# samuelkriegerbonini-dev/AstroBurst

Hardware: AMD Instinct MI355X
Metric: MPix/s sigma-clipped stack+stretch, 64x4096x4096 f32 (higher is better)
Workload: dtype f32

## Files before the change

astroburst_amd/csrc/tile_stream.hpp:

```cpp
#pragma once
#include <hip/hip_runtime.h>

#include <cstdint>

#include "ab_common.hpp"
#include "tile_bucket.hpp"

namespace ts {

using tb::dev_key;
using tb::wave_scan_incl;
using tb::wave_sort64;
using tb::Window;

constexpr int kThreads = 256;
constexpr int kWaves = kThreads / 64;
constexpr int kBuckets = 4096;
constexpr int kTop = kBuckets - 1;
constexpr int kPer = kBuckets / kThreads;
constexpr int kHotCap = 3072;
constexpr int kTabCap = 384;
constexpr int kSelCap = 1024;
constexpr int kMaxZones = 16;
constexpr int kRing = 2;
constexpr int kRingPlan = 3;
constexpr int kEdgePlan = 12;
#ifndef TS_PER_SIGMA
#define TS_PER_SIGMA 480.0f
#endif
constexpr float kPerSigma = TS_PER_SIGMA;
constexpr unsigned int kNone = 0xffffffffu;

enum Decline {
    D_NONE = 0, D_ZONES, D_HOT_OVERFLOW, D_MED_CATCHALL, D_MED_COLD, D_MED_BIG, D_DEV_BM, D_DEV_NOFIRST, D_DEV_SHAPE, D_DEV_COLD,
    D_DEV_BIG, D_DEV_COUNT, D_DEV_PROOF, D_EDGE_COLD, D_EDGE_CATCHALL, D_SAMPLE
};

struct alignas(16) Shared {
    unsigned int prefix[kBuckets + kThreads];
    float list[kHotCap + kThreads];
    union {
        unsigned char lut[kBuckets];
        unsigned int tmp[kSelCap];
    };
    unsigned int zcur[kMaxZones + kThreads];
    uint32_t tab_first[kTabCap], tab_last[kTabCap];
    unsigned int part[4 * kWaves];
    unsigned int zone_at[kMaxZones + 1];
    int zone_lo[kMaxZones], zone_hi[kMaxZones];
    int zone_tab[kMaxZones];
    int nzones;
    int decline;
    unsigned int ncand;
#ifdef AB_TILE_TIMING
    long long t_phase[16];
    long long t_mark;
#endif
};

#ifdef AB_TILE_TIMING
#define TS_MARK(sh, i)                             \
    do {                                           \
        if (threadIdx.x == 0) {                    \
            const long long now_ = clock64();      \
            (sh).t_phase[i] += now_ - (sh).t_mark; \
            (sh).t_mark = now_;                    \
        }                                          \
    } while (0)
#else
#define TS_MARK(sh, i) \
    do {               \
    } while (0)
#endif

__device__ __forceinline__ uint32_t ord_of(float x) {
    const uint32_t b = __float_as_uint(x);
    return b ^ ((b >> 31) ? 0xffffffffu : 0x80000000u);
}
__device__ __forceinline__ float from_ord(uint32_t u) { return __uint_as_float(u ^ ((u >> 31) ? 0x80000000u : 0xffffffffu)); }

struct Geo {
    float scale, off;
    float r_min, r_max;
    ab_pixel_xf xf;
    double range;
    __device__ __forceinline__ int bucket(float v) const { return (int)__builtin_amdgcn_fmed3f(__builtin_fmaf(v, scale, off), 0.0f, (float)kTop); }
    __device__ __forceinline__ bool is_cand(float v) const { return v >= r_min && v <= r_max; }
    __device__ __forceinline__ uint32_t norm_key(float raw) const { return __float_as_uint(ab_px(xf, raw)); }
    __device__ __forceinline__ float unnorm(float x) const { return xf.on ? (float)((double)x * range + xf.lo) : x; }
    __device__ __forceinline__ int bucket_at_norm(float x) const { return bucket(unnorm(x)); }
    __device__ __forceinline__ bool first_raw(int b, float *out) const {
        uint32_t u = ord_of(((float)b - off) / scale);
        int guard = 0;
        while (bucket(from_ord(u)) >= b && ++guard < 64) --u;
        while (bucket(from_ord(u)) < b && ++guard < 128) ++u;
        *out = from_ord(u);
        return guard < 128 && bucket(from_ord(u)) >= b && bucket(from_ord(u - 1u)) < b;
    }
    __device__ __forceinline__ bool first_norm(int b, uint32_t *key) const {
        if (b <= 0) {
            *key = 0x33d6bf96u;
            return true;
        }
        float r;
        if (!first_raw(b, &r)) return false;
        *key = norm_key(r < r_min ? r_min : r);
        return true;
    }
    __device__ __forceinline__ bool last_norm(int b, uint32_t *key) const {
        if (b >= kTop) {
            *key = norm_key(r_max);
            return true;
        }
        float r;
        if (!first_raw(b + 1, &r)) return false;
        r = from_ord(ord_of(r) - 1u);
        *key = norm_key(r < r_min ? r_min : r);
        return true;
    }
};

__device__ __forceinline__ void scan_prefix(Shared &sh) {
    const int t = threadIdx.x, b0 = t * kPer, w = t >> 6, lane = t & 63;
    unsigned int v[kPer];
#pragma unroll
    for (int j = 0; j < kPer; j += 4) {
        const uint4 q = *reinterpret_cast<const uint4 *>(&sh.prefix[b0 + j]);
        v[j] = q.x;
        v[j + 1] = q.y;
        v[j + 2] = q.z;
        v[j + 3] = q.w;
    }
#pragma unroll
    for (int j = 1; j < kPer; ++j) v[j] += v[j - 1];
    const unsigned int tot = v[kPer - 1], incl = wave_scan_incl(tot);
    if (lane == 63) sh.part[w] = incl;
    __syncthreads();
    unsigned int before = incl - tot;
#pragma unroll
    for (int i = 0; i < kWaves; ++i) before += i < w ? sh.part[i] : 0u;
#pragma unroll
    for (int j = 0; j < kPer; j += 4) {
        uint4 q;
        q.x = v[j] + before;
        q.y = v[j + 1] + before;
        q.z = v[j + 2] + before;
        q.w = v[j + 3] + before;
        *reinterpret_cast<uint4 *>(&sh.prefix[b0 + j]) = q;
    }
    __syncthreads();
}

__device__ __forceinline__ void wave_sync() { __builtin_amdgcn_fence(__ATOMIC_ACQ_REL, "wavefront"); }
__device__ __forceinline__ int first_lane(unsigned long long m) { return (int)__builtin_ctzll(m); }
__device__ __forceinline__ unsigned int lanes_below(unsigned long long m) {
    return __builtin_amdgcn_mbcnt_hi((unsigned int)(m >> 32), __builtin_amdgcn_mbcnt_lo((unsigned int)m, 0u));
}
__device__ __forceinline__ unsigned int below(const Shared &sh, int b) { return b <= 0 ? 0u : sh.prefix[b - 1]; }

__device__ __forceinline__ int wfind_rank(const Shared &sh, unsigned int g) {
    const int lane = threadIdx.x & 63;
    const unsigned long long m1 = __builtin_amdgcn_ballot_w64(g < sh.prefix[64 * lane + 63]);
    const int L = m1 ? first_lane(m1) : 63;
    const unsigned long long m2 = __builtin_amdgcn_ballot_w64(g < sh.prefix[64 * L + lane]);
    return 64 * L + (m2 ? first_lane(m2) : 63);
}

__device__ __forceinline__ unsigned int wprefix(const Shared &sh, const Window &w, int b) {
    const unsigned int p = below(sh, b);
    const unsigned int q = p < w.c_lo ? w.c_lo : (p > w.c_le_hi ? w.c_le_hi : p);
    return q - w.c_lo;
}

struct ZReg {
    int lo, hi, tab;
    unsigned int at, end;
    int n;
    __device__ __forceinline__ void load(const Shared &sh) {
        const int lane = threadIdx.x & 63;
        n = sh.nzones;
        const bool have = lane < n;
        lo = have ? sh.zone_lo[lane] : 0;
        hi = have ? sh.zone_hi[lane] : -1;
        tab = have ? sh.zone_tab[lane] : -1;
        at = have ? sh.zone_at[lane] : 0u;
        end = have ? sh.zone_at[lane + 1] : 0u;
    }
    __device__ __forceinline__ int zone_of(int b) const {
        const unsigned long long m = __builtin_amdgcn_ballot_w64(b >= lo && b <= hi);
        return m ? first_lane(m) : -1;
    }
    __device__ __forceinline__ int lo_of(int z) const { return __builtin_amdgcn_readlane(lo, z); }
    __device__ __forceinline__ int hi_of(int z) const { return __builtin_amdgcn_readlane(hi, z); }
    __device__ __forceinline__ unsigned int at_of(int z) const { return (unsigned int)__builtin_amdgcn_readlane((int)at, z); }
    __device__ __forceinline__ unsigned int end_of(int z) const { return (unsigned int)__builtin_amdgcn_readlane((int)end, z); }
    __device__ __forceinline__ int tab_index(int b) const {
        const unsigned long long m = __builtin_amdgcn_ballot_w64(tab >= 0 && b >= lo - 1 && b <= hi + 1);
        if (!m) return -1;
        const int z = first_lane(m);
        return __builtin_amdgcn_readlane(tab, z) + (b - __builtin_amdgcn_readlane(lo, z) + 1);
    }
};
__device__ __forceinline__ bool tfirst(const Shared &sh, const ZReg &zr, const Geo &g, int b, uint32_t *key) {
    const int i = zr.tab_index(b);
    if (i < 0) return g.first_norm(b, key);
    *key = sh.tab_first[i];
    return *key != 0u;
}
__device__ __forceinline__ bool tlast(const Shared &sh, const ZReg &zr, const Geo &g, int b, uint32_t *key) {
    const int i = zr.tab_index(b);
    if (i < 0) return g.last_norm(b, key);
    *key = sh.tab_last[i];
    return *key != 0u;
}

struct DevGeo {
    float mf;
    float delta;
    int bm;
};
__device__ __forceinline__ void ring_of(const Geo &g, const DevGeo &d, float t, int *bl, int *br) {
    const int l = g.bucket_at_norm(d.mf - t), r = g.bucket_at_norm(d.mf + t);
    *bl = l < d.bm ? l : d.bm;
    *br = r > d.bm ? r : d.bm;
}
__device__ __forceinline__ bool make_devgeo(const Shared &sh, const ZReg &zr, const Geo &g, double median, DevGeo *d) {
    d->mf = (float)median;
    int b = g.bucket_at_norm(d->mf), guard = 0;
    uint32_t k;
    auto first_le = [&](int bb, bool *le) {
        if (!tfirst(sh, zr, g, bb, &k)) return false;
        *le = (double)__uint_as_float(k) <= median;
        return true;
    };
    bool le;
    while (b > 0) {
        if (!first_le(b, &le)) return false;
        if (le || ++guard > 8) break;
        --b;
    }
    while (b < kTop) {
        if (!first_le(b + 1, &le)) return false;
        if (!le || ++guard > 16) break;
        ++b;
    }
    d->bm = b;
    if (b <= 0 || b >= kTop || guard > 16) return false;
    uint32_t k0, k1;
    if (!tfirst(sh, zr, g, b, &k0) || !tfirst(sh, zr, g, b + 1, &k1)) return false;
    d->delta = __uint_as_float(k1) - __uint_as_float(k0);
    return d->delta > 0.0f;
}

__device__ __forceinline__ unsigned int wmad_first(const Shared &sh, const Geo &g, const Window &w, const DevGeo &d, unsigned int need, unsigned int guess) {
    const int lane = threadIdx.x & 63;
    auto reaches = [&](unsigned int i) {
        int bl, br;
        ring_of(g, d, (float)(i + 1u) * d.delta, &bl, &br);
        return wprefix(sh, w, br + 1) - wprefix(sh, w, bl) >= need;
    };
    if (guess != kNone) {
        const unsigned int gi = guess < 3900u ? guess : 3900u, i_lo = gi > 96u ? gi - 96u : 0u;
#pragma unroll 1
        for (int j = 0; j < 4; ++j) {
            const unsigned long long m = __builtin_amdgcn_ballot_w64(reaches(i_lo + 64u * j + lane));
            if (m) {
                const unsigned int first = i_lo + 64u * j + (unsigned int)first_lane(m);
                if (first > i_lo || i_lo == 0u) return first;
                break;
            }
        }
    }
#pragma unroll 1
    for (int j = 0; j < kBuckets / 64; ++j) {
        const unsigned long long m = __builtin_amdgcn_ballot_w64(reaches(64u * j + lane));
        if (m) return 64u * j + (unsigned int)first_lane(m);
    }
    return kNone;
}

__device__ __forceinline__ int plan_zones(Shared &sh, const Geo &g, unsigned int cnt, float mad_guess, unsigned int (&first_guess)[3]) {
    int nz = 0;
    auto add = [&](int lo, int hi) {
        lo = lo < 1 ? 1 : lo;
        hi = hi > kTop - 1 ? kTop - 1 : hi;
        if (lo <= hi && nz < kMaxZones) {
            if ((threadIdx.x & 63) == 0) {
                sh.zone_lo[nz] = lo;
                sh.zone_hi[nz] = hi;
            }
            ++nz;
        }
    };
    Window w;
    w.lo = 1;
    w.hi = 0x7f7fffffu;
    w.c_lo = 0;
    w.c_le_hi = cnt;
    w.n = cnt;
    first_guess[0] = first_guess[1] = first_guess[2] = kNone;
#pragma unroll 1
    for (int it = 0; it < 3; ++it) {
        if (w.n < 3) break;
        const unsigned int mid = w.n / 2, g_hi = w.c_lo + mid, g_lo = w.n % 2 == 0 ? g_hi - 1 : g_hi;
        const int b_hi = wfind_rank(sh, g_hi), b_lo = g_lo == g_hi ? b_hi : wfind_rank(sh, g_lo);
        add(b_lo - 1, b_hi + 1);
        if (b_hi <= 0 || b_hi >= kTop) break;
        uint32_t k0, k1;
        if (!g.first_norm(b_hi, &k0) || !g.first_norm(b_hi + 1, &k1)) break;
        const unsigned int ex = below(sh, b_hi), in_b = sh.prefix[b_hi] - ex;
        const float frac = ((float)(g_hi - ex) + 0.5f) / (float)(in_b ? in_b : 1u);
        const float v0 = __uint_as_float(k0), v1 = __uint_as_float(k1);
        const double med = (double)(v0 + frac * (v1 - v0));
        DevGeo d;
        d.mf = (float)med;
        d.bm = b_hi;
        d.delta = v1 - v0;
        if (!(d.delta > 0.0f)) break;
        unsigned int guess = kNone;
        if (it == 0) {
            if (mad_guess > 0.0f) {
                const float gi = mad_guess / d.delta;
                guess = gi < 3900.0f ? (unsigned int)gi : 3900u;
            }
        } else {
            guess = first_guess[it - 1];
        }
        const unsigned int first = wmad_first(sh, g, w, d, mid + 1u, guess);
        if (first == kNone) break;
        first_guess[it] = first;
        {
            int bLo, bRo, bLi = d.bm, bRi = d.bm;
            ring_of(g, d, (float)(first + 1u + kRing + kRingPlan) * d.delta, &bLo, &bRo);
            if (first + 1u > (unsigned int)(kRing + kRingPlan)) ring_of(g, d, (float)(first + 1u - kRing - kRingPlan) * d.delta, &bLi, &bRi);
            if (bLi + 1 >= bRi) {
                add(bLo, bRo);
            } else {
                add(bLo, bLi);
                add(bRi, bRo);
            }
        }
        if (it == 2) break;
        const double mad = (double)(((float)first + 0.5f) * d.delta);
        const double sig = fmax(mad * 1.4826, 1e-30);
        const float lo = (float)(med - 3.0 * sig), hi = (float)(med + 3.0 * sig);
        if (!(lo <= hi)) break;
        const float e = (float)kEdgePlan * d.delta;
        int bl = 0, bh = kTop;
        if (lo > 0.0f) {
            add(g.bucket_at_norm(lo - e), g.bucket_at_norm(lo + e));
            bl = g.bucket_at_norm(lo);
        }
        if (hi < 3.0e38f) {
            add(g.bucket_at_norm(hi - e), g.bucket_at_norm(hi + e));
            bh = g.bucket_at_norm(hi);
        }
        unsigned int c_lo = lo > 0.0f ? below(sh, bl) + (sh.prefix[bl] - below(sh, bl)) / 2u : 0u;
        unsigned int c_hi = hi < 3.0e38f ? sh.prefix[bh] - (sh.prefix[bh] - below(sh, bh)) / 2u : cnt;
        c_lo = c_lo > w.c_lo ? c_lo : w.c_lo;
        c_hi = c_hi < w.c_le_hi ? c_hi : w.c_le_hi;
        if (c_hi <= c_lo) break;
        w.c_lo = c_lo;
        w.c_le_hi = c_hi;
        w.n = c_hi - c_lo;
    }
    return nz;
}

__device__ __forceinline__ bool build_zones(Shared &sh, const Geo &g, int nz) {
    const int lane = threadIdx.x & 63;
    wave_sync();
    uint32_t key = lane < nz ? ((uint32_t)sh.zone_lo[lane] << 16) | (uint32_t)sh.zone_hi[lane] : kNone;
    key = wave_sort64(key);
    int m = 0, cur_lo = 0, cur_hi = -2;
    int my_lo = 0, my_hi = -1;
    for (int i = 0; i < nz; ++i) {
        const uint32_t k = (uint32_t)__builtin_amdgcn_readlane((int)key, i);
        const int lo = (int)(k >> 16), hi = (int)(k & 0xffffu);
        if (m > 0 && lo <= cur_hi + 1) {
            cur_hi = hi > cur_hi ? hi : cur_hi;
        } else {
            if (m > 0 && lane == m - 1) {
                my_lo = cur_lo;
                my_hi = cur_hi;
            }
            cur_lo = lo;
            cur_hi = hi;
            ++m;
        }
    }
    if (m > 0 && lane == m - 1) {
        my_lo = cur_lo;
        my_hi = cur_hi;
    }
    const unsigned int size = lane < m ? sh.prefix[my_hi] - below(sh, my_lo) : 0u;
    const unsigned int tlen = lane < m ? (unsigned int)(my_hi - my_lo + 3) : 0u;
    const unsigned int at = wave_scan_incl(size) - size, tat = wave_scan_incl(tlen) - tlen;
    if (lane < m) {
        sh.zone_lo[lane] = my_lo;
        sh.zone_hi[lane] = my_hi;
        sh.zone_at[lane] = at;
        sh.zcur[lane] = at;
        sh.zone_tab[lane] = tat + tlen <= (unsigned int)kTabCap ? (int)tat : -1;
        if (lane == m - 1) sh.zone_at[m] = at + size;
    }
    if (lane == 0) sh.nzones = m;
    wave_sync();
    return m != 0 && sh.zone_at[m] <= (unsigned int)kHotCap;
}
__device__ __forceinline__ void fill_zone_tables(Shared &sh, const Geo &g) {
    const int t = threadIdx.x, m = sh.nzones;
    for (int z = 0; z < m; ++z) {
        const int lo = sh.zone_lo[z], hi = sh.zone_hi[z], tb0 = sh.zone_tab[z];
        for (int b = lo + t; b <= hi; b += kThreads) sh.lut[b] = (unsigned char)(z + 1);
        if (tb0 >= 0)
            for (int b = lo - 1 + t; b <= hi + 1; b += kThreads) {
                uint32_t kf = 0u, kl = 0u;
                if (!g.first_norm(b, &kf)) kf = 0u;
                if (!g.last_norm(b, &kl)) kl = 0u;
                sh.tab_first[tb0 + (b - lo + 1)] = kf;
                sh.tab_last[tb0 + (b - lo + 1)] = kl;
            }
    }
}

__device__ __forceinline__ void wselect2(Shared &sh, unsigned int n, unsigned int r_lo, unsigned int r_hi, uint32_t *k_lo, uint32_t *k_hi) {
    constexpr int kMine = kSelCap / 64;
    const int lane = threadIdx.x & 63;
    unsigned int *const hist = &sh.prefix[kBuckets];
    wave_sync();
    if (n <= 64u) {
        const uint32_t sorted = wave_sort64((unsigned int)lane < n ? sh.tmp[lane] : kNone);
        *k_lo = (uint32_t)__builtin_amdgcn_readlane((int)sorted, (int)r_lo);
        *k_hi = (uint32_t)__builtin_amdgcn_readlane((int)sorted, (int)r_hi);
        return;
    }
    uint32_t mine[kMine];
    const uint32_t k0 = sh.tmp[0];
    uint32_t diff = 0;
#pragma unroll
    for (int q = 0; q < kMine; ++q) {
        const unsigned int i = (unsigned int)(q * 64 + lane);
        mine[q] = i < n ? sh.tmp[i] : k0;
        diff |= mine[q] ^ k0;
    }
#pragma unroll
    for (int off = 32; off >= 1; off >>= 1) diff |= (uint32_t)__shfl_xor((int)diff, off, 64);
    int top = 24;
    while (top > 0 && (diff >> top) == 0) top -= 8;
    uint32_t mask = top == 24 ? 0u : (0xffffffffu << (top + 8));
    uint32_t prefix = k0 & mask;
    unsigned int rank = r_hi;
    for (int shift = top; shift >= 0; shift -= 8) {
        *reinterpret_cast<uint4 *>(&hist[4 * lane]) = make_uint4(0u, 0u, 0u, 0u);
        wave_sync();
#pragma unroll
        for (int q = 0; q < kMine; ++q)
            if ((unsigned int)(q * 64) < n) {
                if ((unsigned int)(q * 64 + lane) < n && (mine[q] & mask) == prefix) atomicAdd(&hist[(mine[q] >> shift) & 255u], 1u);
            }
        wave_sync();
        const uint4 c = *reinterpret_cast<const uint4 *>(&hist[4 * lane]);
        const unsigned int own = c.x + c.y + c.z + c.w;
        const unsigned int incl = wave_scan_incl(own);
        const unsigned int excl = incl - own;
        const bool owner = rank >= excl && rank < incl;
        uint32_t digit = 0;
        unsigned int bel = 0;
        if (owner) {
            const unsigned int r = rank - excl;
            if (r < c.x) {
                digit = 4 * lane;
                bel = excl;
            } else if (r < c.x + c.y) {
                digit = 4 * lane + 1;
                bel = excl + c.x;
            } else if (r < c.x + c.y + c.z) {
                digit = 4 * lane + 2;
                bel = excl + c.x + c.y;
            } else {
                digit = 4 * lane + 3;
                bel = excl + c.x + c.y + c.z;
            }
        }
        const unsigned long long om = __builtin_amdgcn_ballot_w64(owner);
        const int ol = om ? first_lane(om) : 0;
        digit = (uint32_t)__builtin_amdgcn_readlane((int)digit, ol);
        bel = (unsigned int)__builtin_amdgcn_readlane((int)bel, ol);
        rank -= bel;
        prefix |= digit << shift;
        mask |= 255u << shift;
    }
    *k_hi = prefix;
    *k_lo = prefix;
    if (r_lo != r_hi && rank == 0) {
        uint32_t best = 0;
#pragma unroll
        for (int q = 0; q < kMine; ++q)
            if ((unsigned int)(q * 64 + lane) < n && mine[q] < prefix) best = best > mine[q] ? best : mine[q];
        *k_lo = tb::wave_max(best);
    }
}

template <class KeyOf>
__device__ __forceinline__ unsigned int gather_keys(Shared &sh, unsigned int from, unsigned int to, uint32_t k_from, uint32_t k_to, unsigned int at,
                                                    KeyOf key_of) {
    const int lane = threadIdx.x & 63;
    const uint32_t *const list = reinterpret_cast<const uint32_t *>(sh.list);
#pragma unroll 1
    for (unsigned int i0 = from; i0 < to; i0 += 256) {
        uint32_t key[4];
#pragma unroll
        for (int j = 0; j < 4; ++j) {
            const unsigned int i = i0 + 64u * j + lane;
            const uint32_t k = i < to ? list[i] : 0u;
            key[j] = (k >= k_from && k <= k_to) ? key_of(k) : kNone;
        }
#pragma unroll
        for (int j = 0; j < 4; ++j) {
            const unsigned long long m = __builtin_amdgcn_ballot_w64(key[j] != kNone);
            const unsigned int pos = at + lanes_below(m);
            if (key[j] != kNone && pos < (unsigned int)kSelCap) sh.tmp[pos] = key[j];
            at += (unsigned int)__builtin_popcountll(m);
        }
        if (at > (unsigned int)kSelCap) return kNone;
    }
    return at;
}

struct Rounds {
    Shared &sh;
    const Geo &g;
    ZReg zr;
    __device__ __forceinline__ bool fail(int why) {
        sh.decline = why;
        return false;
    }
    __device__ __forceinline__ bool key_range(int ba, int bb, uint32_t *k_from, uint32_t *k_to) {
        uint32_t prev, next;
        if (!tfirst(sh, zr, g, ba, k_from) || !tlast(sh, zr, g, bb, k_to) || !tlast(sh, zr, g, ba - 1, &prev) || !tfirst(sh, zr, g, bb + 1, &next)) return false;
        if (prev >= *k_from && sh.prefix[ba - 1] != below(sh, ba - 1)) return false;
        if (next <= *k_to && sh.prefix[bb + 1] != sh.prefix[bb]) return false;
        return true;
    }
    __device__ __forceinline__ bool select_values(unsigned int g_lo, unsigned int g_hi, uint32_t *k_lo, uint32_t *k_hi) {
        const int b_hi = wfind_rank(sh, g_hi), b_lo = g_lo == g_hi ? b_hi : wfind_rank(sh, g_lo);
        if (b_lo <= 0 || b_hi >= kTop) return fail(D_MED_CATCHALL);
        const int z_lo = zr.zone_of(b_lo), z_hi = zr.zone_of(b_hi);
        if (z_lo < 0 || z_hi < 0) return fail(D_MED_COLD);
        auto same = [](uint32_t k) { return k; };
        uint32_t kf, kt;
        if (!key_range(b_lo, b_lo, &kf, &kt)) return fail(D_MED_COLD);
        unsigned int n = gather_keys(sh, zr.at_of(z_lo), zr.end_of(z_lo), kf, kt, 0u, same);
        if (n != kNone && b_hi != b_lo) {
            if (!key_range(b_hi, b_hi, &kf, &kt)) return fail(D_MED_COLD);
            n = gather_keys(sh, zr.at_of(z_hi), zr.end_of(z_hi), kf, kt, n, same);
        }
        if (n == kNone) return fail(D_MED_BIG);
        const unsigned int ex = below(sh, b_lo);
        if (n != sh.prefix[b_hi] - ex) return fail(D_MED_COLD);
        TS_MARK(sh, 8);
        wselect2(sh, n, g_lo - ex, g_hi - ex, k_lo, k_hi);
        TS_MARK(sh, 9);
        return true;
    }
    __device__ __forceinline__ bool select_devs(const Window &w, double median, unsigned int r_lo, unsigned int r_hi, unsigned int guess, uint32_t *d_lo,
                                                uint32_t *d_hi) {
        DevGeo d;
        if (!make_devgeo(sh, zr, g, median, &d)) return fail(D_DEV_BM);
        TS_MARK(sh, 10);
        const unsigned int first = wmad_first(sh, g, w, d, r_hi + 1u, guess);
        TS_MARK(sh, 11);
        if (first == kNone) return fail(D_DEV_NOFIRST);
        int bLo, bRo, bLi = 0, bRi = 0;
        ring_of(g, d, (float)(first + 1u + kRing) * d.delta, &bLo, &bRo);
        const bool has_inner_t = first + 1u > (unsigned int)kRing;
        if (has_inner_t) ring_of(g, d, (float)(first + 1u - kRing) * d.delta, &bLi, &bRi);
        const bool has_inner = has_inner_t && bLi + 1 <= bRi - 1;
        const unsigned int c_in = has_inner ? wprefix(sh, w, bRi) - wprefix(sh, w, bLi + 1) : 0u;
        const unsigned int n_cand = wprefix(sh, w, bRo + 1) - wprefix(sh, w, bLo) - c_in;
        if (!(bLo > 0 && bRo < kTop && c_in <= r_lo && c_in + n_cand >= r_hi + 1u && n_cand <= (unsigned int)kSelCap)) return fail(D_DEV_SHAPE);
        auto key_of = [&](uint32_t k) { return (k >= w.lo && k <= w.hi) ? dev_key(k, median) : kNone; };
        unsigned int n;
        uint32_t kf, kt;
        if (has_inner) {
            const int zl = zr.zone_of(bLo), zq = zr.zone_of(bRi);
            if (zl < 0 || zq < 0 || bLi > zr.hi_of(zl) || bRo > zr.hi_of(zq)) return fail(D_DEV_COLD);
            if (!key_range(bLo, bLi, &kf, &kt)) return fail(D_DEV_COLD);
            n = gather_keys(sh, zr.at_of(zl), zr.end_of(zl), kf, kt, 0u, key_of);
            if (n != kNone) {
                if (!key_range(bRi, bRo, &kf, &kt)) return fail(D_DEV_COLD);
                n = gather_keys(sh, zr.at_of(zq), zr.end_of(zq), kf, kt, n, key_of);
            }
        } else {
            const int z = zr.zone_of(bLo);
            if (z < 0 || bRo > zr.hi_of(z)) return fail(D_DEV_COLD);
            if (!key_range(bLo, bRo, &kf, &kt)) return fail(D_DEV_COLD);
            n = gather_keys(sh, zr.at_of(z), zr.end_of(z), kf, kt, 0u, key_of);
        }
        if (n == kNone) return fail(D_DEV_BIG);
        if (n != n_cand) return fail(D_DEV_COUNT);
        TS_MARK(sh, 12);
        uint32_t sel_lo, sel_hi;
        wselect2(sh, n, r_lo - c_in, r_hi - c_in, &sel_lo, &sel_hi);
        TS_MARK(sh, 13);
        uint32_t t_in = 0, t_out = kNone;
        if (has_inner) {
            uint32_t ka, kb;
            if (!tfirst(sh, zr, g, bLi + 1, &ka) || !tlast(sh, zr, g, bRi - 1, &kb)) return fail(D_DEV_PROOF);
            ka = ka > w.lo ? ka : w.lo;
            kb = kb < w.hi ? kb : w.hi;
            if (ka <= kb) {
                const uint32_t da = dev_key(ka, median), db = dev_key(kb, median);
                t_in = da > db ? da : db;
            }
        }
        if (wprefix(sh, w, bLo) > 0u) {
            uint32_t k;
            if (!tlast(sh, zr, g, bLo - 1, &k) || !((double)__uint_as_float(k) <= median)) return fail(D_DEV_PROOF);
            t_out = dev_key(k, median);
        }
        if (wprefix(sh, w, kBuckets) - wprefix(sh, w, bRo + 1) > 0u) {
            uint32_t k;
            if (!tfirst(sh, zr, g, bRo + 1, &k) || !((double)__uint_as_float(k) >= median)) return fail(D_DEV_PROOF);
            const uint32_t dd = dev_key(k, median);
            t_out = t_out < dd ? t_out : dd;
        }
        TS_MARK(sh, 14);
        if (!(t_in <= sel_lo && sel_hi <= t_out)) return fail(D_DEV_PROOF);
        *d_lo = sel_lo;
        *d_hi = sel_hi;
        return true;
    }
    template <bool HI>
    __device__ __forceinline__ bool count_edge(uint32_t bound, unsigned int *out) {
        const int lane = threadIdx.x & 63;
        int b = g.bucket_at_norm(__uint_as_float(bound)), guard = 0;
        auto reaches = [&](int bb, bool *r) {
            uint32_t k;
            if (!tlast(sh, zr, g, bb, &k)) return false;
            *r = HI ? k > bound : k >= bound;
            return true;
        };
        bool r;
        while (b > 0) {
            if (!reaches(b - 1, &r)) return fail(D_EDGE_COLD);
            if (!r || ++guard > 8) break;
            --b;
        }
        while (b < kTop) {
            if (!reaches(b, &r)) return fail(D_EDGE_COLD);
            if (r || ++guard > 16) break;
            ++b;
        }
        if (guard > 16) return fail(D_EDGE_COLD);
        const unsigned int bel = below(sh, b), in_b = sh.prefix[b] - bel;
        if (in_b == 0) {
            *out = bel;
            return true;
        }
        if (b <= 0 || b >= kTop) {
            uint32_t kf, kl;
            if (!tfirst(sh, zr, g, b, &kf) || !tlast(sh, zr, g, b, &kl)) return fail(D_EDGE_CATCHALL);
            if (HI ? kl <= bound : kl < bound) {
                *out = bel + in_b;
                return true;
            }
            if (HI ? kf > bound : kf >= bound) {
                *out = bel;
                return true;
            }
            return fail(D_EDGE_CATCHALL);
        }
        const int z = zr.zone_of(b);
        uint32_t kf, kt;
        if (z < 0 || !key_range(b, b, &kf, &kt)) return fail(D_EDGE_COLD);
        const uint32_t *const list = reinterpret_cast<const uint32_t *>(sh.list);
        unsigned int c = 0, seen = 0;
        const unsigned int to = zr.end_of(z);
        for (unsigned int i0 = zr.at_of(z); i0 < to; i0 += 256) {
#pragma unroll
            for (int j = 0; j < 4; ++j) {
                const unsigned int i = i0 + 64u * j + lane;
                const uint32_t k = i < to ? list[i] : 0u;
                const bool mine = k >= kf && k <= kt;
                seen += mine ? 1u : 0u;
                c += (mine && (HI ? k <= bound : k < bound)) ? 1u : 0u;
            }
        }
        seen = tb::wave_sum(seen);
        c = tb::wave_sum(c);
        if (seen != in_b) return fail(D_EDGE_COLD);
        *out = bel + c;
        return true;
    }

    __device__ __forceinline__ bool run(unsigned int cnt, const unsigned int (&first_guess)[3], double *median_out, double *sigma_out) {
        constexpr double kMadToSigma = 1.4826;
        zr.load(sh);
        Window w;
        w.lo = 1;
        w.hi = 0x7f7fffffu;
        w.c_lo = 0;
        w.c_le_hi = cnt;
        w.n = cnt;
        double median = 0.0, sigma = 1.0;
#pragma unroll 1
        for (int it = 0; it < 3; ++it) {
            if (it < 2 && w.n < 3) continue;
            if (w.n == 0) {
                median = 0.0;
                sigma = 1.0;
                break;
            }
            const unsigned int mid = w.n / 2;
            uint32_t ka, kb;
            if (!select_values(w.c_lo + (w.n % 2 == 0 ? mid - 1 : mid), w.c_lo + mid, &ka, &kb)) return false;
            median = w.n % 2 == 0 ? ((double)__uint_as_float(ka) + (double)__uint_as_float(kb)) / 2.0 : (double)__uint_as_float(kb);
            uint32_t da, db;
            if (!select_devs(w, median, w.n % 2 == 0 ? mid - 1 : mid, mid, first_guess[it], &da, &db)) return false;
            const float mad_f32 = w.n % 2 == 0 ? (__uint_as_float(da) + __uint_as_float(db)) / 2.0f : __uint_as_float(db);
            const double sig = fmax((double)mad_f32 * kMadToSigma, 1e-30);
            if (it == 2) {
                sigma = sig;
                break;
            }
            const float lo = (float)(median - 3.0 * sig), hi = (float)(median + 3.0 * sig);
            if (!(lo <= hi)) {
                w.n = 0;
                w.c_lo = w.c_le_hi = 0;
                w.lo = 1;
                w.hi = 0;
                continue;
            }
            const uint32_t klo = lo > 0.0f ? __float_as_uint(lo) : 1u;
            const uint32_t khi = hi > 0.0f ? (__float_as_uint(hi) > 0x7f7fffffu ? 0x7f7fffffu : __float_as_uint(hi)) : 0u;
            const bool new_lo = klo > w.lo, new_hi = khi < w.hi;
            w.lo = new_lo ? klo : w.lo;
            w.hi = new_hi ? khi : w.hi;
            if (w.lo > w.hi) {
                w.n = 0;
                w.c_lo = w.c_le_hi = 0;
                continue;
            }
            TS_MARK(sh, 6);
            if (new_lo && w.lo > 0x33d6bf96u && !count_edge<false>(w.lo, &w.c_lo)) return false;
            if (new_hi && !count_edge<true>(w.hi, &w.c_le_hi)) return false;
            w.n = w.c_le_hi - w.c_lo;
            TS_MARK(sh, 15);
        }
        *median_out = median;
        *sigma_out = sigma;
        return true;
    }
};

struct TileRect {
    const float *img;
    int64_t ld;
    int y0, y1, x0, x1;
    bool vec;
};
struct __attribute__((packed, aligned(4))) F4u {
    float x, y, z, w;
};
__device__ __forceinline__ float4 load4u(const float *p) {
    const F4u t = *reinterpret_cast<const F4u *>(p);
    return make_float4(t.x, t.y, t.z, t.w);
}
__device__ __forceinline__ bool whole_tile(const TileRect &r) { return r.vec && r.y1 - r.y0 == 256 && r.x1 - r.x0 == 256; }
template <class F>
__device__ __forceinline__ void stream_whole_tile_batches(const TileRect &r, F f) {
    constexpr int U = 4, kRounds = 64 / (2 * U);
    const int t = threadIdx.x, lane = t & 63, wv = t >> 6;
    const float *p = r.img + (int64_t)(r.y0 + wv) * r.ld + r.x0 + 4 * lane;
    const int64_t step = (int64_t)kWaves * r.ld;
    float4 A[U], B[U];
    auto load = [&](float4(&X)[U]) {
#pragma unroll
        for (int u = 0; u < U; ++u) X[u] = load4u(p + u * step);
        p += U * step;
    };
    unsigned int at = (unsigned int)(wv * 256 + 4 * lane);
    auto eat = [&](const float4(&X)[U]) {
        float v[4 * U];
#pragma unroll
        for (int u = 0; u < U; ++u) {
            v[4 * u + 0] = X[u].x;
            v[4 * u + 1] = X[u].y;
            v[4 * u + 2] = X[u].z;
            v[4 * u + 3] = X[u].w;
        }
        f(v, at);
        at += (unsigned int)(U * kWaves * 256);
    };
    load(A);
#pragma unroll 1
    for (int it = 0; it < kRounds; ++it) {
        load(B);
        eat(A);
        if (it + 1 < kRounds) load(A);
        eat(B);
    }
}
template <class F>
__device__ __forceinline__ void stream_tile(const TileRect &r, F f) {
    const int t = threadIdx.x;
    if (whole_tile(r)) {
        constexpr int U = 4, kRounds = 64 / (2 * U);
        const int lane = t & 63, wv = t >> 6;
        const float *p = r.img + (int64_t)(r.y0 + wv) * r.ld + r.x0 + 4 * lane;
        const int64_t step = (int64_t)kWaves * r.ld;
        float4 A[U], B[U];
        auto load = [&](float4(&X)[U]) {
#pragma unroll
            for (int u = 0; u < U; ++u) X[u] = load4u(p + u * step);
            p += U * step;
        };
        auto eat = [&](const float4(&X)[U]) {
#pragma unroll
            for (int u = 0; u < U; ++u) {
                f(X[u].x);
                f(X[u].y);
                f(X[u].z);
                f(X[u].w);
            }
        };
        load(A);
#pragma unroll 1
        for (int it = 0; it < kRounds; ++it) {
            load(B);
            eat(A);
            if (it + 1 < kRounds) load(A);
            eat(B);
        }
    } else if (r.vec) {
        constexpr int U = 8;
        const int lane = t & 63, wv = t >> 6, c = r.x0 + 4 * lane;
        const bool col_ok = c < r.x1;
        const float *p = r.img + c;
#pragma unroll 1
        for (int r0 = r.y0 + wv; r0 < r.y1; r0 += kWaves * U) {
            float4 raw[U];
#pragma unroll
            for (int u = 0; u < U; ++u) {
                const int row = r0 + kWaves * u;
                raw[u] = (col_ok && row < r.y1) ? load4u(p + (int64_t)row * r.ld)
                                                : make_float4(__builtin_nanf(""), __builtin_nanf(""), __builtin_nanf(""), __builtin_nanf(""));
            }
#pragma unroll
            for (int u = 0; u < U; ++u) {
                f(raw[u].x);
                f(raw[u].y);
                f(raw[u].z);
                f(raw[u].w);
            }
        }
    } else {
        constexpr int U = 16;
        const int c = r.x0 + t;
        const bool col_ok = c < r.x1;
        const float *p = r.img + c;
#pragma unroll 1
        for (int r0 = r.y0; r0 < r.y1; r0 += U) {
            float raw[U];
#pragma unroll
            for (int u = 0; u < U; ++u) raw[u] = (col_ok && r0 + u < r.y1) ? p[(int64_t)(r0 + u) * r.ld] : __builtin_nanf("");
#pragma unroll
            for (int u = 0; u < U; ++u) f(raw[u]);
        }
    }
}

struct TileResult {
    double median, sigma;
    int valid;
    int declined;
};

__device__ __forceinline__ void candidate_range(const ab_pixel_xf &xf, float *r_min, float *r_max) {
    if (!xf.on) {
        *r_min = __uint_as_float(0x33d6bf96u);
        *r_max = 3.4028234663852886e38f;
        return;
    }
    *r_max = __builtin_inff();
    uint32_t lo = ord_of(-__builtin_inff()), hi = ord_of(__builtin_inff());
    while (hi - lo > 1u) {
        const uint32_t mid = lo + ((hi - lo) >> 1);
        if (ab_px(xf, from_ord(mid)) > 1e-7f)
            hi = mid;
        else
            lo = mid;
    }
    *r_min = from_ord(hi);
}

__device__ __forceinline__ bool zoom_from_sample(Shared &sh, const TileRect &r, const ab_pixel_xf &xf, Geo *g, float *mad_guess) {
    const int t = threadIdx.x, lane = t & 63, wv = t >> 6;
    const int h = r.y1 - r.y0, wd = r.x1 - r.x0;
    g->xf = xf;
    g->range = xf.on ? 1.0 / xf.inv : 1.0;
    candidate_range(xf, &g->r_min, &g->r_max);
    const int sr = r.y0 + (int)(((unsigned int)t * (unsigned int)h) >> 8), sc = r.x0 + (int)(((unsigned int)(t * 67 + 13) % 256u * (unsigned int)wd) >> 8);
    const float sv = r.img[(int64_t)sr * r.ld + sc];
    const uint32_t sorted = wave_sort64(g->is_cand(sv) ? ord_of(sv) : 0u);
    const int nz = __builtin_popcountll(__builtin_amdgcn_ballot_w64(sorted == 0u)), nv = 64 - nz;
    const uint32_t q1 = (uint32_t)__shfl((int)sorted, nz + nv / 4 < 64 ? nz + nv / 4 : 63, 64);
    const uint32_t q2 = (uint32_t)__shfl((int)sorted, nz + nv / 2 < 64 ? nz + nv / 2 : 63, 64);
    const uint32_t q3 = (uint32_t)__shfl((int)sorted, nz + (3 * nv) / 4 < 64 ? nz + (3 * nv) / 4 : 63, 64);
    if (lane == 0) {
        sh.part[4 * wv + 0] = q1;
        sh.part[4 * wv + 1] = q2;
        sh.part[4 * wv + 2] = q3;
        sh.part[4 * wv + 3] = nv >= 8 ? 1u : 0u;
    }
    __syncthreads();
    float s1 = 0.0f, s2 = 0.0f, s3 = 0.0f, sn = 0.0f;
#pragma unroll
    for (int i = 0; i < kWaves; ++i) {
        const bool ok = sh.part[4 * i + 3] != 0u;
        s1 += ok ? from_ord(sh.part[4 * i + 0]) : 0.0f;
        s2 += ok ? from_ord(sh.part[4 * i + 1]) : 0.0f;
        s3 += ok ? from_ord(sh.part[4 * i + 2]) : 0.0f;
        sn += ok ? 1.0f : 0.0f;
    }
    __syncthreads();
    if (!(sn > 0.0f)) return false;
    const float Q1 = s1 / sn, Q2 = s2 / sn, Q3 = s3 / sn;
    const float sig = (Q3 - Q1) * (1.0f / 1.349f);
    const float wb = sig / kPerSigma;
    g->scale = 1.0f / wb;
    const float vlo = Q2 - (float)((kBuckets - 2) / 2) * wb;
    g->off = 1.0f - vlo * g->scale;
    *mad_guess = 0.6745f * sig * (float)(xf.on ? xf.inv : 1.0);
    return sig > 0.0f && __builtin_isfinite(g->scale) && __builtin_isfinite(g->off) && g->scale > 0.0f;
}

struct CandSink {
    uint2 *ent = nullptr;
    unsigned int *cnt = nullptr;
    float *cut = nullptr;
    unsigned int cap = 0;
};
#ifndef TS_CAND_SIGMAS
#define TS_CAND_SIGMAS 2.5f
#endif
constexpr float kCandSigmas = TS_CAND_SIGMAS;

__device__ __forceinline__ int rounds_wave() {
#ifdef TS_ROUNDS_WAVE0
    return 0;
#else
    return (int)(blockIdx.x & 3u);
#endif
}

__device__ __forceinline__ TileResult tile_stats(Shared &sh, const TileRect &r, const ab_pixel_xf &xf, const CandSink cs = CandSink()) {
    const int t = threadIdx.x;
    TileResult res = {0.0, 1.0, 0, 0};
    if (cs.cut && t == 0) {
        *cs.cut = __builtin_nanf("");
        *cs.cnt = 0u;
    }
#ifdef AB_TILE_TIMING
    if (t == 0) {
        for (int i = 0; i < 16; ++i) sh.t_phase[i] = 0;
        sh.t_mark = clock64();
    }
#endif
    if (t == 0) {
        sh.decline = D_NONE;
        sh.nzones = 0;
        sh.ncand = 0u;
    }
#pragma unroll
    for (int i = 0; i < kPer; i += 4) *reinterpret_cast<uint4 *>(&sh.prefix[t * kPer + i]) = make_uint4(0u, 0u, 0u, 0u);
    *reinterpret_cast<uint4 *>(&sh.lut[16 * t]) = make_uint4(0u, 0u, 0u, 0u);
    Geo g;
    float mad_guess;
    if (!zoom_from_sample(sh, r, xf, &g, &mad_guess)) {
        res.declined = D_SAMPLE;
        return res;
    }
    TS_MARK(sh, 0);
    stream_tile(r, [&](float v) { atomicAdd(&sh.prefix[g.is_cand(v) ? g.bucket(v) : kBuckets + t], 1u); });
    __syncthreads();
    TS_MARK(sh, 1);
    scan_prefix(sh);
    const unsigned int cnt = sh.prefix[kTop];
    TS_MARK(sh, 2);
    if (cnt < 8) return res;
    res.valid = 1;
    unsigned int first_guess[3] = {kNone, kNone, kNone};
    const int rw = rounds_wave();
    if ((t >> 6) == rw) {
        const int nz = plan_zones(sh, g, cnt, mad_guess, first_guess);
        TS_MARK(sh, 3);
        if (!build_zones(sh, g, nz)) sh.decline = sh.nzones == 0 ? D_ZONES : D_HOT_OVERFLOW;
    }
    __syncthreads();
    if (sh.decline) {
        res.declined = sh.decline;
        return res;
    }
    fill_zone_tables(sh, g);
    __syncthreads();
    TS_MARK(sh, 4);
    const int cb = (kBuckets - 2) / 2 + 1 + (int)(kCandSigmas * kPerSigma);
    float cut_raw = 0.0f;
    const bool emit = cs.ent != nullptr && cb > 1 && cb < kTop && whole_tile(r) && g.first_raw(cb, &cut_raw);
    if (whole_tile(r)) {
        stream_whole_tile_batches(r, [&](const float(&v)[16], unsigned int pos0) {
            int b[16];
            unsigned int z[16], at[16];
#pragma unroll
            for (int i = 0; i < 16; ++i) b[i] = g.bucket(v[i]);
#pragma unroll
            for (int i = 0; i < 16; ++i) z[i] = sh.lut[b[i]];
#pragma unroll
            for (int i = 0; i < 16; ++i) z[i] = g.is_cand(v[i]) ? z[i] : 0u;
#pragma unroll
            for (int i = 0; i < 16; ++i) at[i] = atomicAdd(&sh.zcur[z[i] ? z[i] - 1u : (unsigned int)(kMaxZones + t)], 1u);
#pragma unroll
            for (int i = 0; i < 16; ++i) sh.list[(z[i] && at[i] < (unsigned int)kHotCap) ? at[i] : (unsigned int)(kHotCap + t)] = v[i];
            if (emit) {
                unsigned int hit = 0;
#pragma unroll
                for (int i = 0; i < 16; ++i) hit |= (b[i] >= cb && v[i] <= g.r_max) ? 1u << i : 0u;
                while (hit) {
                    const int i = __builtin_ctz(hit);
                    hit &= hit - 1u;
                    const unsigned int ca = atomicAdd(&sh.ncand, 1u);
                    float vi = v[0];
#pragma unroll
                    for (int k = 1; k < 16; ++k) vi = i == k ? v[k] : vi;
                    if (ca < cs.cap) cs.ent[ca] = make_uint2(pos0 + (unsigned int)((i >> 2) * (kWaves * 256) + (i & 3)), __float_as_uint(vi));
                }
            }
        });
    } else {
        stream_tile(r, [&](float v) {
            unsigned int z = sh.lut[g.bucket(v)];
            z = g.is_cand(v) ? z : 0u;
            const unsigned int at = atomicAdd(&sh.zcur[z ? z - 1u : (unsigned int)(kMaxZones + t)], 1u);
            sh.list[(z && at < (unsigned int)kHotCap) ? at : (unsigned int)(kHotCap + t)] = v;
        });
    }
    __syncthreads();
    if (emit && t == 0) {
        *cs.cnt = sh.ncand;
        *cs.cut = cut_raw;
    }
    {
        const unsigned int n = sh.zone_at[sh.nzones];
        for (unsigned int i = t; i < n; i += kThreads) sh.list[i] = __uint_as_float(g.norm_key(sh.list[i]));
    }
    __syncthreads();
    TS_MARK(sh, 5);
#ifdef AB_TILE_TIMING
    if (t == 0) sh.t_phase[7] = sh.zone_at[sh.nzones] * 1000 + sh.nzones;
#endif
    if ((t >> 6) != rw) return res;
    Rounds rounds = {sh, g, ZReg()};
    if (!rounds.run(cnt, first_guess, &res.median, &res.sigma)) res.declined = sh.decline ? sh.decline : 1;
    TS_MARK(sh, 6);
    return res;
}

}
```

Before: 113,100.

## Pack histogram counts into 16-bit halves with coarse/fine two-level prefix

Replaces the 32-bit per-bucket histogram with packed 16-bit counters (two buckets per word) and stores the scanned prefix as a per-block 32-bit coarse base plus 16-bit fine offsets. This halves the shared-memory footprint of the histogram, which can raise occupancy and reduce LDS traffic in the scan. Every prefix lookup now reads two arrays and adds them. A new decline path is taken when a half-word could overflow, and those tiles fall back to the slower route.

```diff
diff --git a/astroburst_amd/csrc/tile_prefix.hpp b/astroburst_amd/csrc/tile_prefix.hpp
--- /dev/null
+++ b/astroburst_amd/csrc/tile_prefix.hpp
@@ -0,0 +1,28 @@
+#pragma once
+#include <cstdint>
+
+#if defined(__HIPCC__)
+#define AB_TP_HD __host__ __device__ __forceinline__
+#else
+#define AB_TP_HD inline
+#endif
+
+namespace tp {
+
+constexpr int kBuckets = 4096;
+constexpr int kPer = 16;
+constexpr int kBlocks = kBuckets / kPer;
+constexpr int kWords = kBuckets / 2;
+constexpr uint32_t kHalfLimit = 0x10000u;
+
+AB_TP_HD int count_word(int b) { return b >> 1; }
+AB_TP_HD uint32_t count_inc(int b) { return 1u << (16 * (b & 1)); }
+AB_TP_HD int sink_bucket(int t) { return kBuckets + 2 * t; }
+AB_TP_HD uint32_t even_half(uint32_t word) { return word & 0xffffu; }
+AB_TP_HD uint32_t odd_half(uint32_t word) { return word >> 16; }
+AB_TP_HD uint32_t pack_halves(uint32_t even, uint32_t odd) { return (even & 0xffffu) | (odd << 16); }
+AB_TP_HD uint32_t pre(const uint32_t *coarse, const uint16_t *fine, int b) { return coarse[b >> 4] + (uint32_t)fine[b]; }
+AB_TP_HD bool counts_intact(uint32_t counted, uint32_t sunk, uint32_t area) { return area < kHalfLimit || counted + sunk == area; }
+AB_TP_HD bool block_fits(uint32_t block_total) { return block_total < kHalfLimit; }
+
+}
diff --git a/astroburst_amd/csrc/tile_stream.hpp b/astroburst_amd/csrc/tile_stream.hpp
--- a/astroburst_amd/csrc/tile_stream.hpp
+++ b/astroburst_amd/csrc/tile_stream.hpp
@@ -5,6 +5,7 @@
 
 #include "ab_common.hpp"
 #include "tile_bucket.hpp"
+#include "tile_prefix.hpp"
 
 namespace ts {
 
@@ -33,11 +34,16 @@
 
 enum Decline {
     D_NONE = 0, D_ZONES, D_HOT_OVERFLOW, D_MED_CATCHALL, D_MED_COLD, D_MED_BIG, D_DEV_BM, D_DEV_NOFIRST, D_DEV_SHAPE, D_DEV_COLD,
-    D_DEV_BIG, D_DEV_COUNT, D_DEV_PROOF, D_EDGE_COLD, D_EDGE_CATCHALL, D_SAMPLE
+    D_DEV_BIG, D_DEV_COUNT, D_DEV_PROOF, D_EDGE_COLD, D_EDGE_CATCHALL, D_SAMPLE,
+    D_PACKED
 };
 
 struct alignas(16) Shared {
-    unsigned int prefix[kBuckets + kThreads];
+    union {
+        uint32_t cnt[tp::kWords + kThreads];
+        uint16_t fine[kBuckets];
+    };
+    uint32_t coarse[kThreads];
     float list[kHotCap + kThreads];
     union {
         unsigned char lut[kBuckets];
@@ -120,35 +126,55 @@
     }
 };
 
-__device__ __forceinline__ void scan_prefix(Shared &sh) {
-    const int t = threadIdx.x, b0 = t * kPer, w = t >> 6, lane = t & 63;
+__device__ __forceinline__ unsigned int pre(const Shared &sh, int b) { return tp::pre(sh.coarse, sh.fine, b); }
+
+__device__ __forceinline__ bool scan_prefix(Shared &sh, unsigned int area) {
+    static_assert(kPer == tp::kPer && kBuckets == tp::kBuckets && kThreads == tp::kBlocks, "tile_prefix.hpp describes this scan");
+    const int t = threadIdx.x, w0 = t * (kPer / 2), w = t >> 6, lane = t & 63;
     unsigned int v[kPer];
 #pragma unroll
-    for (int j = 0; j < kPer; j += 4) {
-        const uint4 q = *reinterpret_cast<const uint4 *>(&sh.prefix[b0 + j]);
-        v[j] = q.x;
-        v[j + 1] = q.y;
-        v[j + 2] = q.z;
-        v[j + 3] = q.w;
+    for (int j = 0; j < kPer / 2; j += 4) {
+        const uint4 q = *reinterpret_cast<const uint4 *>(&sh.cnt[w0 + j]);
+        v[2 * j + 0] = tp::even_half(q.x);
+        v[2 * j + 1] = tp::odd_half(q.x);
+        v[2 * j + 2] = tp::even_half(q.y);
+        v[2 * j + 3] = tp::odd_half(q.y);
+        v[2 * j + 4] = tp::even_half(q.z);
+        v[2 * j + 5] = tp::odd_half(q.z);
+        v[2 * j + 6] = tp::even_half(q.w);
+        v[2 * j + 7] = tp::odd_half(q.w);
     }
 #pragma unroll
     for (int j = 1; j < kPer; ++j) v[j] += v[j - 1];
     const unsigned int tot = v[kPer - 1], incl = wave_scan_incl(tot);
-    if (lane == 63) sh.part[w] = incl;
+    const unsigned int sunk = tb::wave_sum(sh.cnt[tp::kWords + t]);
+    const bool wide = __builtin_amdgcn_ballot_w64(!tp::block_fits(tot)) != 0ull;
+    if (lane == 63) {
+        sh.part[w] = incl;
+        sh.part[kWaves + w] = sunk;
+        sh.part[2 * kWaves + w] = wide ? 1u : 0u;
+    }
     __syncthreads();
-    unsigned int before = incl - tot;
-#pragma unroll
-    for (int i = 0; i < kWaves; ++i) before += i < w ? sh.part[i] : 0u;
-#pragma unroll
-    for (int j = 0; j < kPer; j += 4) {
+    unsigned int before = incl - tot, counted = 0u, all_sunk = 0u, any_wide = 0u;
+#pragma unroll
+    for (int i = 0; i < kWaves; ++i) {
+        before += i < w ? sh.part[i] : 0u;
+        counted += sh.part[i];
+        all_sunk += sh.part[kWaves + i];
+        any_wide |= sh.part[2 * kWaves + i];
+    }
+    sh.coarse[t] = before;
+#pragma unroll
+    for (int j = 0; j < kPer / 2; j += 4) {
         uint4 q;
-        q.x = v[j] + before;
-        q.y = v[j + 1] + before;
-        q.z = v[j + 2] + before;
-        q.w = v[j + 3] + before;
-        *reinterpret_cast<uint4 *>(&sh.prefix[b0 + j]) = q;
+        q.x = tp::pack_halves(v[2 * j + 0], v[2 * j + 1]);
+        q.y = tp::pack_halves(v[2 * j + 2], v[2 * j + 3]);
+        q.z = tp::pack_halves(v[2 * j + 4], v[2 * j + 5]);
+        q.w = tp::pack_halves(v[2 * j + 6], v[2 * j + 7]);
+        *reinterpret_cast<uint4 *>(&sh.cnt[w0 + j]) = q;
     }
     __syncthreads();
+    return any_wide == 0u && tp::counts_intact(counted, all_sunk, area);
 }
 
 __device__ __forceinline__ void wave_sync() { __builtin_amdgcn_fence(__ATOMIC_ACQ_REL, "wavefront"); }
@@ -156,13 +182,13 @@
 __device__ __forceinline__ unsigned int lanes_below(unsigned long long m) {
     return __builtin_amdgcn_mbcnt_hi((unsigned int)(m >> 32), __builtin_amdgcn_mbcnt_lo((unsigned int)m, 0u));
 }
-__device__ __forceinline__ unsigned int below(const Shared &sh, int b) { return b <= 0 ? 0u : sh.prefix[b - 1]; }
+__device__ __forceinline__ unsigned int below(const Shared &sh, int b) { return b <= 0 ? 0u : pre(sh, b - 1); }
 
 __device__ __forceinline__ int wfind_rank(const Shared &sh, unsigned int g) {
     const int lane = threadIdx.x & 63;
-    const unsigned long long m1 = __builtin_amdgcn_ballot_w64(g < sh.prefix[64 * lane + 63]);
+    const unsigned long long m1 = __builtin_amdgcn_ballot_w64(g < pre(sh, 64 * lane + 63));
     const int L = m1 ? first_lane(m1) : 63;
-    const unsigned long long m2 = __builtin_amdgcn_ballot_w64(g < sh.prefix[64 * L + lane]);
+    const unsigned long long m2 = __builtin_amdgcn_ballot_w64(g < pre(sh, 64 * L + lane));
     return 64 * L + (m2 ? first_lane(m2) : 63);
 }
 
@@ -308,7 +334,7 @@
         if (b_hi <= 0 || b_hi >= kTop) break;
         uint32_t k0, k1;
         if (!g.first_norm(b_hi, &k0) || !g.first_norm(b_hi + 1, &k1)) break;
-        const unsigned int ex = below(sh, b_hi), in_b = sh.prefix[b_hi] - ex;
+        const unsigned int ex = below(sh, b_hi), in_b = pre(sh, b_hi) - ex;
         const float frac = ((float)(g_hi - ex) + 0.5f) / (float)(in_b ? in_b : 1u);
         const float v0 = __uint_as_float(k0), v1 = __uint_as_float(k1);
         const double med = (double)(v0 + frac * (v1 - v0));
@@ -355,8 +381,8 @@
             add(g.bucket_at_norm(hi - e), g.bucket_at_norm(hi + e));
             bh = g.bucket_at_norm(hi);
         }
-        unsigned int c_lo = lo > 0.0f ? below(sh, bl) + (sh.prefix[bl] - below(sh, bl)) / 2u : 0u;
-        unsigned int c_hi = hi < 3.0e38f ? sh.prefix[bh] - (sh.prefix[bh] - below(sh, bh)) / 2u : cnt;
+        unsigned int c_lo = lo > 0.0f ? below(sh, bl) + (pre(sh, bl) - below(sh, bl)) / 2u : 0u;
+        unsigned int c_hi = hi < 3.0e38f ? pre(sh, bh) - (pre(sh, bh) - below(sh, bh)) / 2u : cnt;
         c_lo = c_lo > w.c_lo ? c_lo : w.c_lo;
         c_hi = c_hi < w.c_le_hi ? c_hi : w.c_le_hi;
         if (c_hi <= c_lo) break;
@@ -393,7 +419,7 @@
         my_lo = cur_lo;
         my_hi = cur_hi;
     }
-    const unsigned int size = lane < m ? sh.prefix[my_hi] - below(sh, my_lo) : 0u;
+    const unsigned int size = lane < m ? pre(sh, my_hi) - below(sh, my_lo) : 0u;
     const unsigned int tlen = lane < m ? (unsigned int)(my_hi - my_lo + 3) : 0u;
     const unsigned int at = wave_scan_incl(size) - size, tat = wave_scan_incl(tlen) - tlen;
     if (lane < m) {
@@ -427,7 +453,7 @@
 __device__ __forceinline__ void wselect2(Shared &sh, unsigned int n, unsigned int r_lo, unsigned int r_hi, uint32_t *k_lo, uint32_t *k_hi) {
     constexpr int kMine = kSelCap / 64;
     const int lane = threadIdx.x & 63;
-    unsigned int *const hist = &sh.prefix[kBuckets];
+    unsigned int *const hist = &sh.cnt[tp::kWords];
     wave_sync();
     if (n <= 64u) {
         const uint32_t sorted = wave_sort64((unsigned int)lane < n ? sh.tmp[lane] : kNone);
@@ -539,8 +565,8 @@
     __device__ __forceinline__ bool key_range(int ba, int bb, uint32_t *k_from, uint32_t *k_to) {
         uint32_t prev, next;
         if (!tfirst(sh, zr, g, ba, k_from) || !tlast(sh, zr, g, bb, k_to) || !tlast(sh, zr, g, ba - 1, &prev) || !tfirst(sh, zr, g, bb + 1, &next)) return false;
-        if (prev >= *k_from && sh.prefix[ba - 1] != below(sh, ba - 1)) return false;
-        if (next <= *k_to && sh.prefix[bb + 1] != sh.prefix[bb]) return false;
+        if (prev >= *k_from && pre(sh, ba - 1) != below(sh, ba - 1)) return false;
+        if (next <= *k_to && pre(sh, bb + 1) != pre(sh, bb)) return false;
         return true;
     }
     __device__ __forceinline__ bool select_values(unsigned int g_lo, unsigned int g_hi, uint32_t *k_lo, uint32_t *k_hi) {
@@ -558,7 +584,7 @@
         }
         if (n == kNone) return fail(D_MED_BIG);
         const unsigned int ex = below(sh, b_lo);
-        if (n != sh.prefix[b_hi] - ex) return fail(D_MED_COLD);
+        if (n != pre(sh, b_hi) - ex) return fail(D_MED_COLD);
         TS_MARK(sh, 8);
         wselect2(sh, n, g_lo - ex, g_hi - ex, k_lo, k_hi);
         TS_MARK(sh, 9);
@@ -654,7 +680,7 @@
             ++b;
         }
         if (guard > 16) return fail(D_EDGE_COLD);
-        const unsigned int bel = below(sh, b), in_b = sh.prefix[b] - bel;
+        const unsigned int bel = below(sh, b), in_b = pre(sh, b) - bel;
         if (in_b == 0) {
             *out = bel;
             return true;
@@ -975,7 +1001,8 @@
         sh.ncand = 0u;
     }
 #pragma unroll
-    for (int i = 0; i < kPer; i += 4) *reinterpret_cast<uint4 *>(&sh.prefix[t * kPer + i]) = make_uint4(0u, 0u, 0u, 0u);
+    for (int i = 0; i < kPer / 2; i += 4) *reinterpret_cast<uint4 *>(&sh.cnt[t * (kPer / 2) + i]) = make_uint4(0u, 0u, 0u, 0u);
+    sh.cnt[tp::kWords + t] = 0u;
     *reinterpret_cast<uint4 *>(&sh.lut[16 * t]) = make_uint4(0u, 0u, 0u, 0u);
     Geo g;
     float mad_guess;
@@ -984,11 +1011,17 @@
         return res;
     }
     TS_MARK(sh, 0);
-    stream_tile(r, [&](float v) { atomicAdd(&sh.prefix[g.is_cand(v) ? g.bucket(v) : kBuckets + t], 1u); });
+    stream_tile(r, [&](float v) {
+        const int b = g.is_cand(v) ? g.bucket(v) : tp::sink_bucket(t);
+        atomicAdd(&sh.cnt[tp::count_word(b)], tp::count_inc(b));
+    });
     __syncthreads();
     TS_MARK(sh, 1);
-    scan_prefix(sh);
-    const unsigned int cnt = sh.prefix[kTop];
+    if (!scan_prefix(sh, (unsigned int)((r.y1 - r.y0) * (r.x1 - r.x0)))) {
+        res.declined = D_PACKED;
+        return res;
+    }
+    const unsigned int cnt = pre(sh, kTop);
     TS_MARK(sh, 2);
     if (cnt < 8) return res;
     res.valid = 1;
```

Result: no change. 113,700, median of 3 (+0.5%).
